# christopherkarani/Wax

Measured on NVIDIA H100. Metric: queries/sec cosine top-10 @ 10Mx384 fp32, higher is better.
Workload: dtype f32

## Files before the change

### wax_b200/csrc/waxvs_batch.cuh

```cuda
#pragma once
#include <cuda.h>
#include <cuda_bf16.h>

#include "waxvs_common.cuh"
#include "waxvs_scan.cuh"

namespace waxvs {

constexpr int kBatchM = 128;
constexpr int kBatchN = 128;
constexpr int kBatchKBlock = 32;
constexpr int kBatchKBlockBf16 = 64;
constexpr int kBatchRescore = 256;
constexpr int kBatchRescoreMax = 1024;
constexpr uint32_t kBatchABytes = kBatchM * 128u;
constexpr uint32_t kBatchBBytes = kBatchN * 128u;
constexpr uint32_t kBatchStageBytes = kBatchABytes + kBatchBBytes;
constexpr int kBatchStageSlots = 8;
constexpr uint32_t kBatchScoreStride = kBatchN + 8;
constexpr uint32_t kBatchScoreBytes = kBatchM * kBatchScoreStride * 4u;
constexpr int kBatchMaxStages = 6;
constexpr uint32_t kBatchSmemOptin = 227u * 1024u;
__host__ __device__ constexpr uint32_t batch_smem_bytes(int stages, int heap, uint32_t ares_kb = 0) {
    return ares_kb * kBatchABytes + stages * (ares_kb ? kBatchBBytes : kBatchStageBytes) + kBatchScoreBytes +
// ... 893 lines not shown
            }
        } else if (n_exact >= p.k) {
            const float dk = from_orderable_u32(static_cast<uint32_t>(ek[p.k - 1] >> 32));
            const float qn = s_sqrt_a2;
            const float scale = METRIC == kCosine ? qn : qn * __uint_as_float(*p.max_norm_bits);
            const float sk_exact = METRIC == kCosine ? (1.0f - dk) * qn : 1.0f - dk;
            const float acc_slack = static_cast<float>(p.dims) * 0x1p-23f * scale;
            const float ulp_slack = 0x1p-21f * fmaxf(1.0f, fabsf(dk)) * (METRIC == kCosine ? qn : 1.0f);
            const float eps = p.eps_rel * scale * 1.01f + acc_slack + ulp_slack + 1e-30f;
            if (excluded_any && (!(sk_exact > tau + eps) || !finite_f32(eps))) ok = 0;
            const float feps = kTf32Eps * scale * 1.01f + acc_slack + ulp_slack + 1e-30f;
            const float t = sk_exact - feps;
            tau_star = finite_f32(t) ? t - fabsf(t) * 0x1p-20f - 1e-30f : -INFINITY;
            const float feps16 = kBf16Eps * scale * 1.01f + acc_slack + ulp_slack + 1e-30f;
            const float t16 = sk_exact - feps16;
            tau_star16 = finite_f32(t16) ? t16 - fabsf(t16) * 0x1p-20f - 1e-30f : -INFINITY;
        } else if (excluded_any) {
            ok = 0;
        }
        if (METRIC != kL2 && (!(s_a2 >= 0x1p-126f) || !finite_f32(s_a2))) {
            ok = 0;
            tau_star = tau_star16 = -INFINITY;
        }
        p.ok[q] = ok;
        if (p.tau_star) { p.tau_star[q] = tau_star; p.tau_star[p.tau_stride + q] = tau_star16; }
    }
    ScanParams sp{};
    sp.out = p.out + static_cast<size_t>(q) * p.k;
    sp.frame_ids = p.frame_ids; sp.id_base = p.id_base; sp.row_offset = p.row_offset;
    for (uint32_t i = threadIdx.x; i < p.k; i += blockDim.x)
        write_candidate(sp, static_cast<int>(i), i < p.rescore ? ek[i] : WAXVS_KEY_NONE);
}

struct RescoreParams {
    const float *corpus, *query;
    uint32_t dims, k, n_nominees;
    const uint64_t *nominees;
    uint32_t *aux;
    const uint32_t *max_norm_bits;
    float rho_max;
    uint64_t *block_keys;
    uint32_t *ticket;
    uint32_t *work_counter;
    wax_vs_candidate *out;
    uint32_t *ok;
    const uint64_t *frame_ids;
    uint64_t id_base, row_offset;
    uint32_t tail_smem_bytes;
};

template <int METRIC>
__global__ void __launch_bounds__(512, 1) shadow_rescore_kernel(const RescoreParams p) {
    static_assert(METRIC == kCosine || METRIC == kDot, "the shadow route covers cosine and dot");
    extern __shared__ __align__(16) unsigned char rsm[];
    __shared__ float s_a2, s_sqrt_a2;
    const int warp = threadIdx.x >> 5, lane = threadIdx.x & 31, warps = blockDim.x >> 5;
    const int k = static_cast<int>(p.k);
    if (warp == 0) {
        float s0 = 0.f, s1 = 0.f, s2 = 0.f, s3 = 0.f;
        for (uint32_t base = 4u * lane; base < p.dims; base += 128u) {
            const float4 x = __ldg(reinterpret_cast<const float4 *>(p.query + base));
            s0 = __fmaf_rn(x.x, x.x, s0); s1 = __fmaf_rn(x.y, x.y, s1);
            s2 = __fmaf_rn(x.z, x.z, s2); s3 = __fmaf_rn(x.w, x.w, s3);
        }
        const float a2 = warp_butterfly_sum(__fadd_rn(__fadd_rn(s0, s1), __fadd_rn(s2, s3)));
        if (lane == 0) { s_a2 = a2; s_sqrt_a2 = __fsqrt_rn(a2); }
    }
    __shared__ ScanParams sp;
    for (uint32_t i = threadIdx.x; i < sizeof(ScanParams) / 4u; i += blockDim.x) reinterpret_cast<uint32_t *>(&sp)[i] = 0u;
    __syncthreads();
    if (threadIdx.x == 0) {
        sp.k = p.k; sp.block_keys = p.block_keys; sp.ticket = p.ticket; sp.out = p.out;
        sp.frame_ids = p.frame_ids; sp.id_base = p.id_base; sp.row_offset = p.row_offset;
        sp.tail_smem_bytes = p.tail_smem_bytes; sp.work_counter = p.work_counter;
    }
    __syncthreads();

    WarpTopK<1> tk;
    tk.init();
    const uint32_t stride = gridDim.x * warps * 4u;
    for (uint32_t i0 = (blockIdx.x * warps + warp) * 4u; i0 < p.n_nominees; i0 += stride) {
        uint64_t nk[4];
        const float *vp[4];
        float d[4];
#pragma unroll
        for (uint32_t r = 0; r < 4; ++r) {
            nk[r] = i0 + r < p.n_nominees ? p.nominees[i0 + r] : WAXVS_KEY_NONE;
            vp[r] = p.corpus + static_cast<size_t>(nk[r] == WAXVS_KEY_NONE ? 0u : static_cast<uint32_t>(nk[r])) * p.dims;
        }
        exact_row_distance_x4<METRIC>(p.query, vp, p.dims, s_a2, s_sqrt_a2, lane, d);
#pragma unroll
        for (uint32_t r = 0; r < 4; ++r) {
            if (nk[r] == WAXVS_KEY_NONE || !finite_f32(d[r])) continue;
            const uint64_t x = make_key(d[r], static_cast<uint32_t>(nk[r]));
            if (x < tk.thresh) tk.insert(x, lane, k);
        }
    }

    if (!finish_topk_select<1>(sp, tk, rsm)) return;
    __syncthreads();
    if (threadIdx.x != 0) return;
    const wax_vs_candidate kth = p.out[p.k - 1];
    const uint32_t cut = p.aux[0];
    const bool excluded_any = cut != WAXVS_UKEY_NONE;
    const float tau = excluded_any ? -from_orderable_u32(cut) : -INFINITY;
    const float rho_q = __uint_as_float(p.aux[1]);
    uint32_t ok = 1;
    if (kth.valid) {
        const float dk = kth.distance, qn = s_sqrt_a2;
        const float m = METRIC == kCosine ? 1.0f : __uint_as_float(*p.max_norm_bits);
        const float scale = qn * m;
        const float sk_exact = METRIC == kCosine ? (1.0f - dk) * qn : 1.0f - dk;
        const float coding = qn * p.rho_max + rho_q * ((METRIC == kCosine ? 1.0001f : m) + p.rho_max);
        const float acc_slack = static_cast<float>(p.dims) * 0x1p-23f * scale;
        const float ulp_slack = 0x1p-21f * fmaxf(1.0f, fabsf(dk)) * (METRIC == kCosine ? qn : 1.0f);
        const float eps = coding * 1.01f + acc_slack + ulp_slack + 1e-30f;
        if (excluded_any && (!(sk_exact > tau + eps) || !finite_f32(eps))) ok = 0;
    } else if (excluded_any) {
        ok = 0;
    }
    if (!(s_a2 >= 0x1p-126f) || !finite_f32(s_a2)) ok = 0;
    *p.ok = ok;
    p.aux[0] = WAXVS_UKEY_NONE;
    p.aux[2] = cut;
}

template <int METRIC>
__global__ void __launch_bounds__(256) filter_rescore_kernel(const float *corpus, const float *queries, uint32_t dims,
                                                             const uint32_t *cand_count, const uint32_t *cand_rows,
                                                             uint32_t cand_cap, uint64_t *keys) {
    const uint32_t q = blockIdx.y;
    const int lane = threadIdx.x & 31;
    const uint32_t n = min(cand_count[q], cand_cap);
    const uint32_t warps = (gridDim.x * blockDim.x) >> 5;
    uint32_t i = (blockIdx.x * blockDim.x + threadIdx.x) >> 5;
    if (i >= n) return;
    const float *qv = queries + static_cast<size_t>(q) * dims;
    float a2 = 0.0f, sqrt_a2 = 0.0f;
    if (METRIC == kCosine) {
        float s0 = 0.f, s1 = 0.f, s2 = 0.f, s3 = 0.f;
        for (uint32_t base = 4u * lane; base < dims; base += 128u) {
            const float x = __ldg(qv + base); s0 = __fmaf_rn(x, x, s0);
            if (base + 1 < dims) { const float y = __ldg(qv + base + 1); s1 = __fmaf_rn(y, y, s1); }
            if (base + 2 < dims) { const float z = __ldg(qv + base + 2); s2 = __fmaf_rn(z, z, s2); }
            if (base + 3 < dims) { const float w = __ldg(qv + base + 3); s3 = __fmaf_rn(w, w, s3); }
        }
        a2 = warp_butterfly_sum(__fadd_rn(__fadd_rn(s0, s1), __fadd_rn(s2, s3)));
        sqrt_a2 = __fsqrt_rn(a2);
    }
    for (uint32_t i0 = i; i0 < n; i0 += 4u * warps) {
        uint32_t rr[4];
        const float *vp[4];
        float d[4];
#pragma unroll
        for (uint32_t r = 0; r < 4; ++r) {
            const uint32_t j = i0 + r * warps;
            rr[r] = cand_rows[static_cast<size_t>(q) * cand_cap + (j < n ? j : i0)];
            vp[r] = corpus + static_cast<size_t>(rr[r]) * dims;
        }
// ... 41 lines not shown
```

### wax_b200/csrc/waxvs_engine.cu

```cuda
#include <cuda_runtime.h>

#include <algorithm>
#include <atomic>
#include <cstdarg>
#include <cstdio>
#include <cstring>
#include <mutex>
#include <new>
#include <shared_mutex>
#include <string>
#include <unordered_map>
#include <chrono>
#include <random>
#include <thread>
#include <unistd.h>
#include <cmath>
#include <vector>

#include "../../include/wax_vs_cuda.h"
#include "waxvs_common.cuh"
#include "waxvs_scan.cuh"
#include "waxvs_select.cuh"
#include "waxvs_synth.cuh"
#include "waxvs_batch.cuh"
// ... 523 lines not shown
static cudaError_t launch_shadow_scan(wax_vs_engine *e, const ScanParams &p, int grid, const TmaConfig &cfg, int metric,
                                      cudaStream_t s) {
#define WAXVS_CASE(Cv, Rv)                                                                                          \
    if (cfg.C == Cv && cfg.R == Rv)                                                                                 \
        return metric == kCosine ? launch_tma_inst<Cv, Rv, kCosine, 4, false, true>(e, p, grid, cfg, s)            \
                                 : launch_tma_inst<Cv, Rv, kDot, 4, false, true>(e, p, grid, cfg, s)
    WAXVS_CASE(1, 8); WAXVS_CASE(1, 16); WAXVS_CASE(2, 8); WAXVS_CASE(2, 16);
    WAXVS_CASE(3, 4); WAXVS_CASE(3, 8); WAXVS_CASE(3, 16); WAXVS_CASE(4, 4); WAXVS_CASE(4, 8);
    WAXVS_CASE(6, 2); WAXVS_CASE(6, 4); WAXVS_CASE(8, 2); WAXVS_CASE(8, 4); WAXVS_CASE(12, 2); WAXVS_CASE(12, 4);
#undef WAXVS_CASE
    return cudaErrorInvalidValue;
}
static cudaError_t launch_int8_scan(wax_vs_engine *e, const ScanParams &p, int grid, const TmaConfig &cfg, int metric,
                                   cudaStream_t s) {
#define WAXVS_CASE(Cv, Rv)                                                                                          \
    if (cfg.C == Cv && cfg.R == Rv)                                                                                 \
        return metric == kCosine ? launch_tma_inst<Cv, Rv, kCosine, 4, false, true, true>(e, p, grid, cfg, s)      \
                                 : launch_tma_inst<Cv, Rv, kDot, 4, false, true, true>(e, p, grid, cfg, s)
    WAXVS_CASE(1, 8); WAXVS_CASE(1, 16); WAXVS_CASE(2, 8); WAXVS_CASE(2, 16);
    WAXVS_CASE(3, 4); WAXVS_CASE(3, 8); WAXVS_CASE(3, 16); WAXVS_CASE(4, 4); WAXVS_CASE(4, 8);
    WAXVS_CASE(6, 4); WAXVS_CASE(6, 8); WAXVS_CASE(8, 4); WAXVS_CASE(12, 4);
#undef WAXVS_CASE
    return cudaErrorInvalidValue;
}
static bool pick_u4_config(const wax_vs_engine *e, TmaConfig *cfg) {
    if (!pick_tma_config(e, cfg, 1, 1)) return false;
    const int C = cfg->C, want_r = e->tune.u4_rows_per_step;
    const int r_hi = C <= 3 ? 16 : (C <= 6 ? 8 : 4), r_lo = C <= 3 ? 8 : 4;
    cfg->R = (want_r >= r_lo && want_r <= r_hi && (want_r & (want_r - 1)) == 0) ? want_r : r_hi;
    cfg->stages = e->tune.u4_stages > 0 ? e->tune.u4_stages : 3;
    cfg->warps = std::max(1, std::min(16, e->tune.u4_warps ? e->tune.u4_warps : 16));
    const size_t stage_bytes = static_cast<size_t>(cfg->R) * (e->dims / 2 + 4);
    cfg->smem = static_cast<size_t>(cfg->warps) * cfg->stages * (stage_bytes + 8 + 4) + static_cast<size_t>(cfg->warps) * 1024 + 16;
    return cfg->smem <= (e->smem_optin ? e->smem_optin : 232448) - 4096;
}
static cudaError_t launch_u4_scan(wax_vs_engine *e, const ScanParams &p, int grid, const TmaConfig &cfg, cudaStream_t s) {
#define WAXVS_CASE(Cv, Rv) \
    if (cfg.C == Cv && cfg.R == Rv) return launch_tma_inst<Cv, Rv, kDot, 4, false, true, false, true>(e, p, grid, cfg, s)
    WAXVS_CASE(1, 8); WAXVS_CASE(1, 16); WAXVS_CASE(2, 8); WAXVS_CASE(2, 16); WAXVS_CASE(3, 8); WAXVS_CASE(3, 16);
    WAXVS_CASE(4, 4); WAXVS_CASE(4, 8); WAXVS_CASE(6, 4); WAXVS_CASE(6, 8); WAXVS_CASE(8, 4); WAXVS_CASE(12, 4);
#undef WAXVS_CASE
    return cudaErrorInvalidValue;
}
static cudaError_t launch_ldg(const ScanParams &p, int grid, int metric, int mode, cudaStream_t s) {
    switch (metric * 3 + mode) {
        case 0: scan_ldg_kernel<kCosine, 1, false><<<grid, 256, 0, s>>>(p); break;
        case 1: scan_ldg_kernel<kCosine, 4, false><<<grid, 256, 0, s>>>(p); break;
        case 2: scan_ldg_kernel<kCosine, 1, true><<<grid, 256, 0, s>>>(p); break;
        case 3: scan_ldg_kernel<kDot, 1, false><<<grid, 256, 0, s>>>(p); break;
        case 4: scan_ldg_kernel<kDot, 4, false><<<grid, 256, 0, s>>>(p); break;
        case 5: scan_ldg_kernel<kDot, 1, true><<<grid, 256, 0, s>>>(p); break;
        case 6: scan_ldg_kernel<kL2, 1, false><<<grid, 256, 0, s>>>(p); break;
        case 7: scan_ldg_kernel<kL2, 4, false><<<grid, 256, 0, s>>>(p); break;
        default: scan_ldg_kernel<kL2, 1, true><<<grid, 256, 0, s>>>(p); break;
    }
    return cudaGetLastError();
}

static int32_t wait_host_flag(cudaStream_t stream, unsigned long long *flag_ptr, unsigned long long seq,
                              unsigned long long timeout_ns) {
    volatile unsigned long long *flag = flag_ptr;
    const auto t0 = std::chrono::steady_clock::now();
    uint32_t spins = 0;
    for (;;) {
        const unsigned long long v = *flag;
        if ((v & ~kShardErrorBit) == seq) {
            std::atomic_thread_fence(std::memory_order_acquire);
// ... 94 lines not shown
    *form = RouteForm::kBf16;
    TmaConfig cfg{};
    int32_t rc;
    if (!demoted && e->n_rows * e->dims * sizeof(float) >= e->tune.u4_scan_min_bytes && pick_u4_config(e, &cfg)) {
        if ((rc = ensure_coded_shadow(e, e->u4, stream))) return rc;
        if (e->u4.valid && std::isfinite(e->u4.eps_rel)) { *form = RouteForm::kU4; return WAX_VS_OK; }
    }
    bool int8 = false;
    if ((rc = int8_route_selected(e, stream, &int8))) return rc;
    if (int8) *form = RouteForm::kInt8;
    return WAX_VS_OK;
}

static int32_t enqueue_shadow_nominations(wax_vs_engine *e, SearchCtx *c, const ScanParams &p, const TmaConfig &cfg,
                                          cudaStream_t stream, uint64_t *launches, uint32_t *shape = nullptr,
                                          RouteForm form = RouteForm::kBf16) {
    const bool int8 = form == RouteForm::kInt8, u4 = form == RouteForm::kU4;
    int32_t rc;
    if (u4 && !c->d_u4_aux) {
        if ((rc = c->d_u4_aux.ensure(3, "4-bit route state"))) return rc;
        CUDA_TRY(cudaMemsetAsync(c->d_u4_aux, 0xFF, 3 * sizeof(uint32_t), stream));
    }
    const size_t u4_keys = static_cast<size_t>(std::max(e->tune.grid, e->sm_count)) * kU4CtaNominees;
    if ((rc = c->d_heaps.ensure(std::max(static_cast<size_t>(kShadowNominees) * kNomineeStride, u4 ? u4_keys : 0), "nominee keys")) ||
        (rc = c->d_ok.ensure(1, "proof flags")) || (!p.query && (rc = c->d_queries.ensure(e->dims, "query buffer"))))
        return rc;

    ScanParams sp = p;
    sp.corpus = u4 ? reinterpret_cast<const float *>(e->u4.codes.p)
                   : int8 ? reinterpret_cast<const float *>(e->i8.codes.p) : reinterpret_cast<const float *>(e->d_shadow.p);
    sp.row_scale = u4 ? e->u4.scale.p : int8 ? e->i8.scale.p : nullptr;
    sp.u4_aux = u4 ? c->d_u4_aux.p : nullptr;
    sp.k = kShadowNominees;
    sp.out = nullptr; sp.host_out = nullptr; sp.host_flag = nullptr;
    sp.nominees = c->d_heaps;
    sp.query_store = p.query ? nullptr : c->d_queries.p;
    sp.tail_select = e->tune.tail_select ? 1u : 0u;
    sp.tail_smem_bytes = static_cast<uint32_t>(static_cast<size_t>(cfg.warps) * cfg.stages * cfg.R * e->dims *
                                               (int8 ? 1 : sizeof(__nv_bfloat16)));
    const int grid = tma_grid(e, c, cfg, sp);
    if (u4) CUDA_TRY(launch_u4_scan(e, sp, grid, cfg, stream));
    else if (int8) CUDA_TRY(launch_int8_scan(e, sp, grid, cfg, e->similarity, stream));
    else CUDA_TRY(launch_shadow_scan(e, sp, grid, cfg, e->similarity, stream));

    if (u4) {
        RescoreParams rp{};
        rp.corpus = e->d_corpus; rp.query = p.query ? p.query : c->d_queries.p;
        rp.dims = e->dims; rp.k = p.k; rp.n_nominees = static_cast<uint32_t>(grid) * kU4CtaNominees;
        rp.nominees = c->d_heaps; rp.aux = c->d_u4_aux; rp.max_norm_bits = e->d_max_norm; rp.rho_max = e->u4.rho_max;
        rp.block_keys = c->d_block_keys; rp.ticket = c->d_ticket; rp.work_counter = sp.work_counter; rp.out = p.out; rp.ok = c->d_ok;
        rp.frame_ids = p.frame_ids; rp.id_base = p.id_base; rp.row_offset = p.row_offset;
        rp.tail_smem_bytes = static_cast<uint32_t>(grid) * p.k * sizeof(uint64_t);
        if (rp.tail_smem_bytes > 48u * 1024u) rp.tail_smem_bytes = 0;
        const auto kernel = e->similarity == WAX_VS_COSINE ? shadow_rescore_kernel<kCosine> : shadow_rescore_kernel<kDot>;
        kernel<<<grid, 512, rp.tail_smem_bytes, stream>>>(rp);
        CUDA_TRY(cudaGetLastError());
    } else {
    FinishParams fp{};
    fp.corpus = e->d_corpus; fp.queries = p.query ? p.query : c->d_queries.p;
    fp.n_rows = p.n_rows; fp.dims = e->dims; fp.n_queries = 1; fp.groups = 1; fp.slices = 1;
    fp.kprime = kShadowNominees; fp.k = p.k; fp.metric = e->similarity;
    fp.heaps = c->d_heaps; fp.max_norm_bits = e->d_max_norm;
    fp.out = p.out; fp.ok = c->d_ok;
    fp.frame_ids = p.frame_ids; fp.id_base = p.id_base; fp.row_offset = p.row_offset;
    fp.pow2_all = 512; fp.rescore = kShadowRescore; fp.eps_rel = int8 ? e->i8.eps_rel : kBf16Eps;
    const size_t fsmem = static_cast<size_t>(fp.pow2_all + fp.rescore) * sizeof(uint64_t);
    const auto kernel = e->similarity == WAX_VS_COSINE ? batch_finish_kernel<kCosine> : batch_finish_kernel<kDot>;
    CUDA_TRY(grant_smem(e, kernel, fsmem));
    kernel<<<1, 512, fsmem, stream>>>(fp);
    CUDA_TRY(cudaGetLastError());
    }
    *launches += 2;
    if (shape) {
        const uint32_t s[7] = {static_cast<uint32_t>(cfg.C), static_cast<uint32_t>(cfg.R), static_cast<uint32_t>(cfg.warps),
                               static_cast<uint32_t>(cfg.stages), static_cast<uint32_t>(grid), sp.chunk_steps, sp.tail_select};
        std::copy(s, s + 7, shape);
    }
    return WAX_VS_OK;
}

static int32_t enqueue_shadow_route(wax_vs_engine *e, SearchCtx *c, ScanParams &p, cudaStream_t stream, uint64_t *launches) {
    if (!shadow_route_applies(e)) return WAX_VS_OK;
    TmaConfig cfg{};
    if (!pick_tma_config(e, &cfg, 1, sizeof(__nv_bfloat16))) return WAX_VS_OK;
    int32_t rc;
    if (!c->h_proof_count) {
        if ((rc = c->d_proof_count.ensure(2, "proof counts")) || (rc = c->h_proof_count.ensure(2, "proof count mirror"))) return rc;
        CUDA_TRY(cudaMemsetAsync(c->d_proof_count, 0, 2 * sizeof(uint32_t), stream));
        c->h_proof_count[0] = c->h_proof_count[1] = 0;
        c->seen_failed = 0;
    }
    bool demoted;
    {
        std::lock_guard<std::mutex> pg(e->pool_mu);
        const uint32_t failed = *static_cast<volatile uint32_t *>(c->h_proof_count + 1);
        if (failed != c->seen_failed) {
            c->seen_failed = failed;
            if (c->last_u4) {
                if (e->u4_probing) e->u4_demote_window = std::min(e->u4_demote_window * 2, 1u << 20);
                e->u4_demoted = e->u4_demote_window;
            } else {
                e->shadow_scan_skip = kShadowSkipQueries;
            }
        } else if (c->last_u4 && e->u4_probing) {
            e->u4_demote_window = 16;
// ... 3582 lines not shown
```

### wax_b200/csrc/waxvs_scan.cuh

```cuda
#pragma once
#include "waxvs_common.cuh"
#include "waxvs_shard.cuh"
#include "../../include/wax_vs_cuda.h"

namespace waxvs {

constexpr int kInlineQueryFloats = 512;

struct ScanParams {
    const float *corpus;
    const float *query;
    uint32_t n_rows;
    uint32_t dims;
    uint32_t k;
    uint32_t stages;
    uint64_t *block_keys;
    uint32_t *ticket;
    wax_vs_candidate *out;
    uint32_t *dist_keys;
    const uint64_t *frame_ids;
    uint64_t id_base;
    uint64_t row_offset;
    uint32_t use_l2_hint;
    uint32_t chunk_steps;
    uint32_t *work_counter;
    const uint32_t *mask;
    wax_vs_candidate *host_out;
    unsigned long long *host_flag;
    unsigned long long host_seq;
    alignas(16) float query_inline[kInlineQueryFloats];
    uint32_t tail_select;
    uint32_t tail_smem_bytes;
    unsigned long long *trace;
    ShardParams shard;
    uint64_t *nominees;
    float *query_store;
    const uint32_t *proof_ok;
    uint32_t *proof_count;
    uint32_t *proof_count_host;
    const float *row_scale;
    uint32_t *u4_aux;
};

constexpr uint32_t kU4CtaNominees = 256;

constexpr int kNomineeStride = 128;

__device__ __forceinline__ bool row_allowed(const ScanParams &p, uint32_t row) {
    return p.mask == nullptr || ((__ldg(p.mask + (row >> 5)) >> (row & 31u)) & 1u) != 0u;
}

__device__ __forceinline__ void write_candidate(const ScanParams &p, int slot, uint64_t key) {
    wax_vs_candidate c;
    if (key == WAXVS_KEY_NONE) {
        c.distance = 0.0f; c.valid = 0; c.row = 0; c.frame_id = 0;
    } else {
        const uint32_t row = static_cast<uint32_t>(key);
        c.distance = from_orderable_u32(static_cast<uint32_t>(key >> 32));
        c.valid = 1;
        c.row = p.row_offset + row;
        c.frame_id = p.frame_ids ? p.frame_ids[row] : p.id_base + row;
    }
    p.out[slot] = c;
    if (p.host_out) p.host_out[slot] = c;
}

template <bool SHADOW>
__device__ __forceinline__ void write_slot(const ScanParams &p, int slot, uint64_t key) {
    if constexpr (SHADOW) p.nominees[static_cast<size_t>(slot == static_cast<int>(p.k) - 1 ? 0 : slot + 1) * kNomineeStride] = key;
    else write_candidate(p, slot, key);
}

__device__ __forceinline__ float4 bf16x4_to_float4(uint2 u) {
    return make_float4(__uint_as_float(u.x << 16), __uint_as_float(u.x & 0xFFFF0000u),
                       __uint_as_float(u.y << 16), __uint_as_float(u.y & 0xFFFF0000u));
}

__device__ __forceinline__ float4 int8x4_to_float4(uint32_t u) {
    constexpr float kBias = 8388736.0f;
    return make_float4(__fsub_rn(__uint_as_float(__byte_perm(u, 0x4B000000u, 0x7650)), kBias),
                       __fsub_rn(__uint_as_float(__byte_perm(u, 0x4B000000u, 0x7651)), kBias),
                       __fsub_rn(__uint_as_float(__byte_perm(u, 0x4B000000u, 0x7652)), kBias),
                       __fsub_rn(__uint_as_float(__byte_perm(u, 0x4B000000u, 0x7653)), kBias));
}

template <int H>
__device__ __forceinline__ void half_warp_reduce_scatter(int (&v)[H], int lane) {
    static_assert(H == 1 || H == 2 || H == 4 || H == 8, "H must be a power of two <= 8");
    int off = 8;
#pragma unroll
    for (int half = H / 2; half >= 1; half >>= 1, off >>= 1) {
        const bool upper = (lane & off) != 0;
#pragma unroll
        for (int j = 0; j < half; ++j) {
            const int send = upper ? v[j] : v[j + half];
            const int keep = upper ? v[j + half] : v[j];
            v[j] = keep + __shfl_xor_sync(WAXVS_FULL_MASK, send, off);
        }
    }
#pragma unroll
    for (; off >= 1; off >>= 1) v[0] += __shfl_xor_sync(WAXVS_FULL_MASK, v[0], off);
}

// ... 25 lines not shown
    }
    __syncthreads();
    if (!s_last) return;
    __threadfence();
    tk.init();
    constexpr int U = (E == 1) ? 4 : 2;
#pragma unroll 1
    for (uint32_t b0 = warp; b0 < gridDim.x; b0 += warps * U) {
        uint64_t other[U][E];
#pragma unroll
        for (int u = 0; u < U; ++u) {
            const uint32_t b = b0 + u * warps;
#pragma unroll
            for (int j = 0; j < E; ++j)
                other[u][j] = (b < gridDim.x) ? ld_cg_u64(p.block_keys + static_cast<size_t>(b) * W + j * 32 + lane)
                                              : WAXVS_KEY_NONE;
        }
#pragma unroll
        for (int u = 0; u < U; ++u) tk.merge_sorted(other[u], lane, k);
    }
    __syncthreads();
#pragma unroll
    for (int j = 0; j < E; ++j) lists[warp * W + j * 32 + lane] = tk.key[j];
    __syncthreads();
    if (warp == 0) {
#pragma unroll 1
        for (int w = 1; w < warps; ++w) {
            uint64_t other[E];
            load_list(lists + w * W, other);
            tk.merge_sorted(other, lane, k);
        }
#pragma unroll
        for (int j = 0; j < E; ++j)
            if (j * 32 + lane < k) write_slot<SHADOW>(p, j * 32 + lane, tk.key[j]);
        if (lane == 0) { *p.ticket = 0u; if (p.work_counter) *p.work_counter = 0u; }
        if (p.host_flag && !p.shard.world) {
            __threadfence_system();
            __syncwarp();
            if (lane == 0) st_release_sys_u64(p.host_flag, p.host_seq);
        }
    }
    if (p.shard.world) shard_exchange_cta(p.shard, p.out, p.k, reinterpret_cast<uint32_t *>(lists));
}

struct SelectScratch {
    uint32_t hist[256];
    uint64_t sel[128];
    uint32_t digit, k_rem, in_bin, n_sel;
    unsigned long long found;
};

template <typename ForEach>
__device__ __forceinline__ uint64_t block_select_kth(ForEach for_each, uint32_t k, SelectScratch *ss) {
    const uint32_t tid = threadIdx.x;
    uint64_t prefix = 0;
    uint32_t k_rem = k;
#pragma unroll 1
    for (int shift = 56; shift >= 0; shift -= 8) {
        for (uint32_t i = tid; i < 256u; i += blockDim.x) ss->hist[i] = 0;
        __syncthreads();
        const uint64_t want = (shift == 56) ? 0ull : (prefix >> (shift + 8));
        for_each([&](uint64_t key) {
            if (shift == 56 || (key >> (shift + 8)) == want) atomicAdd(&ss->hist[(key >> shift) & 255u], 1u);
        });
        __syncthreads();
        if (tid < 32) {
            uint32_t c[8], sum = 0;
// ... 1 lines not shown
            for (int i = 0; i < 8; ++i) { c[i] = ss->hist[tid * 8 + i]; sum += c[i]; }
            uint32_t incl = sum;
#pragma unroll
            for (int off = 1; off < 32; off <<= 1) {
                const uint32_t up = __shfl_up_sync(WAXVS_FULL_MASK, incl, off);
                if (static_cast<int>(tid) >= off) incl += up;
            }
            const uint32_t excl = incl - sum;
            if (excl < k_rem && k_rem <= incl) {
                uint32_t run = excl;
#pragma unroll
                for (int i = 0; i < 8; ++i) {
                    if (run < k_rem && k_rem <= run + c[i]) { ss->digit = tid * 8 + i; ss->k_rem = k_rem - run; ss->in_bin = c[i]; }
                    run += c[i];
                }
            }
        }
        __syncthreads();
        prefix |= static_cast<uint64_t>(ss->digit) << shift;
        k_rem = ss->k_rem;
        if (ss->in_bin == 1u && shift > 0) {
            const uint64_t top = prefix >> shift;
            for_each([&](uint64_t key) { if ((key >> shift) == top) ss->found = key; });
            __syncthreads();
            const uint64_t x = ss->found;
            __syncthreads();
            return x;
        }
    }
    return prefix;
}

template <int E, bool SHADOW = false>
__device__ __forceinline__ bool finish_topk_select(const ScanParams &p, WarpTopK<E> &tk, unsigned char *scratch) {
    __shared__ SelectScratch ss;
    __shared__ uint32_t s_last2;
    const uint32_t tid = threadIdx.x, nthr = blockDim.x, k = p.k;
    auto own_keys = [&](auto f) {
#pragma unroll
        for (int j = 0; j < E; ++j) f(tk.key[j]);
    };
    const uint64_t xa = block_select_kth(own_keys, k, &ss);
    if (tid == 0) ss.n_sel = 0;
    __syncthreads();
    uint64_t *mine = p.block_keys + static_cast<size_t>(blockIdx.x) * k;
#pragma unroll
    for (int j = 0; j < E; ++j)
        if (tk.key[j] != WAXVS_KEY_NONE && tk.key[j] <= xa) mine[atomicAdd(&ss.n_sel, 1u)] = tk.key[j];
    __syncthreads();
    for (uint32_t i = ss.n_sel + tid; i < k; i += nthr) mine[i] = WAXVS_KEY_NONE;
    __threadfence();
    __syncthreads();
    if (p.trace && tid == 0) atomicMax(p.trace + 2, global_timer_ns());
    if (tid == 0) s_last2 = (atomicAdd(p.ticket, 1u) == gridDim.x - 1) ? 1u : 0u;
    __syncthreads();
    if (!s_last2) return false;
    __threadfence();
    if (p.trace && tid == 0) p.trace[3] = global_timer_ns();
    const uint32_t total = gridDim.x * k;
    const bool staged = static_cast<size_t>(total) * sizeof(uint64_t) <= p.tail_smem_bytes;
    uint64_t *sk = reinterpret_cast<uint64_t *>(scratch);
    if (staged) {
        for (uint32_t i = tid; i < total; i += nthr) sk[i] = ld_cg_u64(p.block_keys + i);
        __syncthreads();
    }
    auto grid_keys = [&](auto f) {
        if (staged) { for (uint32_t i = tid; i < total; i += nthr) f(sk[i]); }
        else { for (uint32_t i = tid; i < total; i += nthr) f(ld_cg_u64(p.block_keys + i)); }
    };
    const uint64_t xb = block_select_kth(grid_keys, k, &ss);
    if (tid == 0) ss.n_sel = 0;
    __syncthreads();
    grid_keys([&](uint64_t key) { if (key != WAXVS_KEY_NONE && key <= xb) ss.sel[atomicAdd(&ss.n_sel, 1u)] = key; });
    __syncthreads();
    const uint32_t n_sel = ss.n_sel;
    for (uint32_t i = tid; i < k; i += nthr) {
        if (i < n_sel) {
            const uint64_t key = ss.sel[i];
            uint32_t rank = 0;
            for (uint32_t j = 0; j < n_sel; ++j) rank += ss.sel[j] < key ? 1u : 0u;
            write_slot<SHADOW>(p, static_cast<int>(rank), key);
        } else {
            write_slot<SHADOW>(p, static_cast<int>(i), WAXVS_KEY_NONE);
        }
    }
    if (p.host_flag && !p.shard.world) __threadfence_system();
    __syncthreads();
    if (tid == 0) {
        *p.ticket = 0u;
        if (p.work_counter) *p.work_counter = 0u;
        if (p.host_flag && !p.shard.world) st_release_sys_u64(p.host_flag, p.host_seq);
        if (p.trace) p.trace[4] = global_timer_ns();
    }
    if (p.shard.world) shard_exchange_cta(p.shard, p.out, p.k, reinterpret_cast<uint32_t *>(scratch));
    return true;
}

template <int E>
__device__ __forceinline__ void finish_u4_nominees(const ScanParams &p, WarpTopK<E> &tk) {
    __shared__ SelectScratch ss;
    __shared__ uint32_t s_cut;
    const uint32_t tid = threadIdx.x, nthr = blockDim.x;
    if (tid == 0) s_cut = WAXVS_UKEY_NONE;
    auto own_keys = [&](auto f) {
#pragma unroll
        for (int j = 0; j < E; ++j) f(tk.key[j]);
    };
    const uint64_t xa = block_select_kth(own_keys, kU4CtaNominees, &ss);
    if (tid == 0) ss.n_sel = 0;
    __syncthreads();
    uint64_t *mine = p.nominees + static_cast<size_t>(blockIdx.x) * kU4CtaNominees;
#pragma unroll
    for (int j = 0; j < E; ++j)
        if (tk.key[j] != WAXVS_KEY_NONE && tk.key[j] <= xa) mine[atomicAdd(&ss.n_sel, 1u)] = tk.key[j];
    if ((tid & 31u) == 0 && tk.thresh != WAXVS_KEY_NONE) atomicMin(&s_cut, static_cast<uint32_t>(tk.thresh >> 32));
    __syncthreads();
    for (uint32_t i = ss.n_sel + tid; i < kU4CtaNominees; i += nthr) mine[i] = WAXVS_KEY_NONE;
    if (tid == 0) {
        uint32_t cut = s_cut;
        if (xa != WAXVS_KEY_NONE) cut = min(cut, static_cast<uint32_t>(xa >> 32));
        if (cut != WAXVS_UKEY_NONE) atomicMin(p.u4_aux, cut);
    }
}

template <int C, int R, int METRIC, int E, bool EMIT, bool SHADOW = false, bool INT8 = false, bool U4 = false>
__global__ void __launch_bounds__(512, 1) scan_tma_kernel(const __grid_constant__ ScanParams p) {
    static_assert(!SHADOW || (C > 0 && METRIC != kL2 && !EMIT), "the shadow form covers the unrolled cosine / dot shapes");
    static_assert(!INT8 || (SHADOW && R >= 4), "the int8 form is a shadow form with 16-byte scale copies");
    static_assert(!U4 || (SHADOW && !INT8 && R >= 4 && E == 4), "the 4-bit form is a shadow form with 16-byte scale copies");
    constexpr bool SCALED = INT8 || U4;
    if constexpr (!SHADOW && !EMIT && E == 1 && METRIC != kL2) {
        if (p.proof_ok) {
            const bool proven = *p.proof_ok != 0u;
            if (blockIdx.x == 0) {
                if (threadIdx.x == 0) {
                    const uint32_t n = ++p.proof_count[proven ? 0 : 1];
                    *static_cast<volatile uint32_t *>(p.proof_count_host + (proven ? 0 : 1)) = n;
                }
                if (proven && p.host_flag) {
                    for (uint32_t i = threadIdx.x; i < p.k; i += blockDim.x) p.host_out[i] = p.out[i];
                    __threadfence_system();
                    __syncthreads();
                    if (threadIdx.x == 0) st_release_sys_u64(p.host_flag, p.host_seq);
                }
            }
            if (proven) return;
        }
    }
    const int D4 = C > 0 ? 32 * C : static_cast<int>(p.dims / 4u);
    const int CN = C > 0 ? C : (D4 + 31) / 32;
    const uint32_t ROW_BYTES = C > 0 ? (U4 ? 64u : INT8 ? 128u : SHADOW ? 256u : 512u) * C : p.dims * 4u;
    const uint32_t STAGE_BYTES = ROW_BYTES * R + (SCALED ? R * 4u : 0u);
    constexpr int LANES_PER_ROW = 32 / R;

    extern __shared__ __align__(128) unsigned char smem[];
    const int warp = threadIdx.x >> 5, lane = threadIdx.x & 31, warps = blockDim.x >> 5;
    const uint32_t stages = p.stages;
    unsigned char *ring = smem + static_cast<size_t>(warp) * stages * STAGE_BYTES;
    uint64_t *bars = reinterpret_cast<uint64_t *>(smem + static_cast<size_t>(warps) * stages * STAGE_BYTES) +
                     warp * stages;
    uint64_t *lists = reinterpret_cast<uint64_t *>(smem + static_cast<size_t>(warps) * stages * STAGE_BYTES) +
                      warps * stages;
    uint32_t *stage_step = reinterpret_cast<uint32_t *>(lists + warps * 32 * E) + warp * stages;
    float4 *qs = reinterpret_cast<float4 *>(reinterpret_cast<uint32_t *>(lists + warps * 32 * E) + warps * stages + 4);

    float4 q[C > 0 ? C : 1];
    const float4 *q4 = reinterpret_cast<const float4 *>(p.query);
    const float4 *qp = reinterpret_cast<const float4 *>(p.query_inline);
    auto load_q = [&](int i) -> float4 { return q4 ? __ldg(q4 + i) : qp[i]; };
    if (C > 0) {
#pragma unroll
        for (int c = 0; c < (C > 0 ? C : 1); ++c) q[c] = load_q(lane + 32 * c);
// ... 239 lines not shown
        else d = finish_l2(sum0[0]);
        if (SHADOW && !finite_f32(d)) d = -INFINITY;
        const bool leader = U4 ? (hl % (16 / H)) == 0 : (lane % LANES_PER_ROW) == 0;
        const bool ok = (my_row < p.n_rows) && (SHADOW || finite_f32(d));

        if (EMIT) {
            if (leader && my_row < p.n_rows)
                p.dist_keys[my_row] = (ok && row_allowed(p, my_row)) ? orderable_u32(d) : WAXVS_UKEY_NONE;
        } else {
            const uint64_t key = ok ? make_key(d, my_row) : WAXVS_KEY_NONE;
            const bool cand = leader && key < tk.thresh && row_allowed(p, my_row);
            uint32_t m = __ballot_sync(WAXVS_FULL_MASK, cand);
            if (E == 1) {
                while (m) {
                    const int src = __ffs(m) - 1;
                    m &= m - 1;
                    const uint64_t x = shfl_u64(key, src);
                    if (x < tk.thresh) tk.insert(x, lane, k);
                }
            } else if (m) {
                if (tk.npend + __popc(m) > 32) tk.flush(lane, k);
                while (m) {
                    const int src = __ffs(m) - 1;
                    m &= m - 1;
                    tk.park(shfl_u64(key, src), lane);
                }
            }
        }
    }

    if (p.trace && lane == 0) atomicMax(p.trace + 1, global_timer_ns());
    if (!EMIT) {
        if (E > 1) tk.flush(lane, k);
        if constexpr (U4) finish_u4_nominees<E>(p, tk);
        else if (p.tail_select) finish_topk_select<E, SHADOW>(p, tk, smem);
        else finish_topk<E, SHADOW>(p, tk, lists, warp, lane, warps);
    }
}

template <int METRIC, int E, bool EMIT>
__global__ void __launch_bounds__(256, 4) scan_ldg_kernel(const __grid_constant__ ScanParams p) {
    __shared__ uint64_t lists[8 * 32 * E];
    const int warp = threadIdx.x >> 5, lane = threadIdx.x & 31, warps = blockDim.x >> 5;
    const uint32_t dims = p.dims;
    const bool vec4 = (dims % 4u) == 0u;
    const uint32_t d4 = dims / 4u;

    float a2 = 0.0f, sqrt_a2 = 0.0f;
    if (METRIC == kCosine) {
        float s0 = 0.f, s1 = 0.f, s2 = 0.f, s3 = 0.f;
        for (uint32_t base = 4u * lane; base < dims; base += 128u) {
            const float x = __ldg(p.query + base);
            const float y = (base + 1 < dims) ? __ldg(p.query + base + 1) : 0.0f;
            const float z = (base + 2 < dims) ? __ldg(p.query + base + 2) : 0.0f;
            const float w = (base + 3 < dims) ? __ldg(p.query + base + 3) : 0.0f;
            s0 = __fmaf_rn(x, x, s0);
            if (base + 1 < dims) s1 = __fmaf_rn(y, y, s1);
            if (base + 2 < dims) s2 = __fmaf_rn(z, z, s2);
            if (base + 3 < dims) s3 = __fmaf_rn(w, w, s3);
        }
        a2 = warp_butterfly_sum(__fadd_rn(__fadd_rn(s0, s1), __fadd_rn(s2, s3)));
        sqrt_a2 = __fsqrt_rn(a2);
    }

    WarpTopK<E> tk;
    tk.init();
    const int k = static_cast<int>(p.k);
    const uint32_t total_warps = gridDim.x * warps;
// ... 57 lines not shown
```

Baseline: 1499.

## Fuse u4 shadow rescore into scan kernel tail with TMA row gather

```diff
diff --git a/wax_b200/csrc/waxvs_batch.cuh b/wax_b200/csrc/waxvs_batch.cuh
--- a/wax_b200/csrc/waxvs_batch.cuh
+++ b/wax_b200/csrc/waxvs_batch.cuh
@@ -949,99 +949,6 @@
         write_candidate(sp, static_cast<int>(i), i < p.rescore ? ek[i] : WAXVS_KEY_NONE);
 }
 
-struct RescoreParams {
-    const float *corpus, *query;
-    uint32_t dims, k, n_nominees;
-    const uint64_t *nominees;
-    uint32_t *aux;
-    const uint32_t *max_norm_bits;
-    float rho_max;
-    uint64_t *block_keys;
-    uint32_t *ticket;
-    uint32_t *work_counter;
-    wax_vs_candidate *out;
-    uint32_t *ok;
-    const uint64_t *frame_ids;
-    uint64_t id_base, row_offset;
-    uint32_t tail_smem_bytes;
-};
-
-template <int METRIC>
-__global__ void __launch_bounds__(512, 1) shadow_rescore_kernel(const RescoreParams p) {
-    static_assert(METRIC == kCosine || METRIC == kDot, "the shadow route covers cosine and dot");
-    extern __shared__ __align__(16) unsigned char rsm[];
-    __shared__ float s_a2, s_sqrt_a2;
-    const int warp = threadIdx.x >> 5, lane = threadIdx.x & 31, warps = blockDim.x >> 5;
-    const int k = static_cast<int>(p.k);
-    if (warp == 0) {
-        float s0 = 0.f, s1 = 0.f, s2 = 0.f, s3 = 0.f;
-        for (uint32_t base = 4u * lane; base < p.dims; base += 128u) {
-            const float4 x = __ldg(reinterpret_cast<const float4 *>(p.query + base));
-            s0 = __fmaf_rn(x.x, x.x, s0); s1 = __fmaf_rn(x.y, x.y, s1);
-            s2 = __fmaf_rn(x.z, x.z, s2); s3 = __fmaf_rn(x.w, x.w, s3);
-        }
-        const float a2 = warp_butterfly_sum(__fadd_rn(__fadd_rn(s0, s1), __fadd_rn(s2, s3)));
-        if (lane == 0) { s_a2 = a2; s_sqrt_a2 = __fsqrt_rn(a2); }
-    }
-    __shared__ ScanParams sp;
-    for (uint32_t i = threadIdx.x; i < sizeof(ScanParams) / 4u; i += blockDim.x) reinterpret_cast<uint32_t *>(&sp)[i] = 0u;
-    __syncthreads();
-    if (threadIdx.x == 0) {
-        sp.k = p.k; sp.block_keys = p.block_keys; sp.ticket = p.ticket; sp.out = p.out;
-        sp.frame_ids = p.frame_ids; sp.id_base = p.id_base; sp.row_offset = p.row_offset;
-        sp.tail_smem_bytes = p.tail_smem_bytes; sp.work_counter = p.work_counter;
-    }
-    __syncthreads();
-
-    WarpTopK<1> tk;
-    tk.init();
-    const uint32_t stride = gridDim.x * warps * 4u;
-    for (uint32_t i0 = (blockIdx.x * warps + warp) * 4u; i0 < p.n_nominees; i0 += stride) {
-        uint64_t nk[4];
-        const float *vp[4];
-        float d[4];
-#pragma unroll
-        for (uint32_t r = 0; r < 4; ++r) {
-            nk[r] = i0 + r < p.n_nominees ? p.nominees[i0 + r] : WAXVS_KEY_NONE;
-            vp[r] = p.corpus + static_cast<size_t>(nk[r] == WAXVS_KEY_NONE ? 0u : static_cast<uint32_t>(nk[r])) * p.dims;
-        }
-        exact_row_distance_x4<METRIC>(p.query, vp, p.dims, s_a2, s_sqrt_a2, lane, d);
-#pragma unroll
-        for (uint32_t r = 0; r < 4; ++r) {
-            if (nk[r] == WAXVS_KEY_NONE || !finite_f32(d[r])) continue;
-            const uint64_t x = make_key(d[r], static_cast<uint32_t>(nk[r]));
-            if (x < tk.thresh) tk.insert(x, lane, k);
-        }
-    }
-
-    if (!finish_topk_select<1>(sp, tk, rsm)) return;
-    __syncthreads();
-    if (threadIdx.x != 0) return;
-    const wax_vs_candidate kth = p.out[p.k - 1];
-    const uint32_t cut = p.aux[0];
-    const bool excluded_any = cut != WAXVS_UKEY_NONE;
-    const float tau = excluded_any ? -from_orderable_u32(cut) : -INFINITY;
-    const float rho_q = __uint_as_float(p.aux[1]);
-    uint32_t ok = 1;
-    if (kth.valid) {
-        const float dk = kth.distance, qn = s_sqrt_a2;
-        const float m = METRIC == kCosine ? 1.0f : __uint_as_float(*p.max_norm_bits);
-        const float scale = qn * m;
-        const float sk_exact = METRIC == kCosine ? (1.0f - dk) * qn : 1.0f - dk;
-        const float coding = qn * p.rho_max + rho_q * ((METRIC == kCosine ? 1.0001f : m) + p.rho_max);
-        const float acc_slack = static_cast<float>(p.dims) * 0x1p-23f * scale;
-        const float ulp_slack = 0x1p-21f * fmaxf(1.0f, fabsf(dk)) * (METRIC == kCosine ? qn : 1.0f);
-        const float eps = coding * 1.01f + acc_slack + ulp_slack + 1e-30f;
-        if (excluded_any && (!(sk_exact > tau + eps) || !finite_f32(eps))) ok = 0;
-    } else if (excluded_any) {
-        ok = 0;
-    }
-    if (!(s_a2 >= 0x1p-126f) || !finite_f32(s_a2)) ok = 0;
-    *p.ok = ok;
-    p.aux[0] = WAXVS_UKEY_NONE;
-    p.aux[2] = cut;
-}
-
 template <int METRIC>
 __global__ void __launch_bounds__(256) filter_rescore_kernel(const float *corpus, const float *queries, uint32_t dims,
                                                              const uint32_t *cand_count, const uint32_t *cand_rows,
diff --git a/wax_b200/csrc/waxvs_engine.cu b/wax_b200/csrc/waxvs_engine.cu
--- a/wax_b200/csrc/waxvs_engine.cu
+++ b/wax_b200/csrc/waxvs_engine.cu
@@ -579,7 +579,8 @@
     cfg->warps = std::max(1, std::min(16, e->tune.u4_warps ? e->tune.u4_warps : 16));
     const size_t stage_bytes = static_cast<size_t>(cfg->R) * (e->dims / 2 + 4);
     cfg->smem = static_cast<size_t>(cfg->warps) * cfg->stages * (stage_bytes + 8 + 4) + static_cast<size_t>(cfg->warps) * 1024 + 16;
-    return cfg->smem <= (e->smem_optin ? e->smem_optin : 232448) - 4096;
+    return cfg->warps * cfg->stages * stage_bytes >= e->dims * sizeof(float) &&
+           cfg->smem <= (e->smem_optin ? e->smem_optin : 232448) - 12288;
 }
 static cudaError_t launch_u4_scan(wax_vs_engine *e, const ScanParams &p, int grid, const TmaConfig &cfg, cudaStream_t s) {
 #define WAXVS_CASE(Cv, Rv) \
@@ -740,30 +741,24 @@
     sp.row_scale = u4 ? e->u4.scale.p : int8 ? e->i8.scale.p : nullptr;
     sp.u4_aux = u4 ? c->d_u4_aux.p : nullptr;
     sp.k = kShadowNominees;
-    sp.out = nullptr; sp.host_out = nullptr; sp.host_flag = nullptr;
     sp.nominees = c->d_heaps;
-    sp.query_store = p.query ? nullptr : c->d_queries.p;
     sp.tail_select = e->tune.tail_select ? 1u : 0u;
-    sp.tail_smem_bytes = static_cast<uint32_t>(static_cast<size_t>(cfg.warps) * cfg.stages * cfg.R * e->dims *
-                                               (int8 ? 1 : sizeof(__nv_bfloat16)));
+    if (u4) {
+        sp.u4_rows = e->d_corpus; sp.u4_k = p.k; sp.u4_cosine = e->similarity == WAX_VS_COSINE ? 1u : 0u;
+        sp.max_norm_bits = e->d_max_norm; sp.rho_max = e->u4.rho_max; sp.u4_ok = c->d_ok;
+        sp.tail_smem_bytes = static_cast<uint32_t>(cfg.warps * cfg.stages * cfg.R * (e->dims / 2 + 4));
+    } else {
+        sp.out = nullptr; sp.host_out = nullptr; sp.host_flag = nullptr;
+        sp.query_store = p.query ? nullptr : c->d_queries.p;
+        sp.tail_smem_bytes = static_cast<uint32_t>(static_cast<size_t>(cfg.warps) * cfg.stages * cfg.R * e->dims *
+                                                   (int8 ? 1 : sizeof(__nv_bfloat16)));
+    }
     const int grid = tma_grid(e, c, cfg, sp);
     if (u4) CUDA_TRY(launch_u4_scan(e, sp, grid, cfg, stream));
     else if (int8) CUDA_TRY(launch_int8_scan(e, sp, grid, cfg, e->similarity, stream));
     else CUDA_TRY(launch_shadow_scan(e, sp, grid, cfg, e->similarity, stream));
 
-    if (u4) {
-        RescoreParams rp{};
-        rp.corpus = e->d_corpus; rp.query = p.query ? p.query : c->d_queries.p;
-        rp.dims = e->dims; rp.k = p.k; rp.n_nominees = static_cast<uint32_t>(grid) * kU4CtaNominees;
-        rp.nominees = c->d_heaps; rp.aux = c->d_u4_aux; rp.max_norm_bits = e->d_max_norm; rp.rho_max = e->u4.rho_max;
-        rp.block_keys = c->d_block_keys; rp.ticket = c->d_ticket; rp.work_counter = sp.work_counter; rp.out = p.out; rp.ok = c->d_ok;
-        rp.frame_ids = p.frame_ids; rp.id_base = p.id_base; rp.row_offset = p.row_offset;
-        rp.tail_smem_bytes = static_cast<uint32_t>(grid) * p.k * sizeof(uint64_t);
-        if (rp.tail_smem_bytes > 48u * 1024u) rp.tail_smem_bytes = 0;
-        const auto kernel = e->similarity == WAX_VS_COSINE ? shadow_rescore_kernel<kCosine> : shadow_rescore_kernel<kDot>;
-        kernel<<<grid, 512, rp.tail_smem_bytes, stream>>>(rp);
-        CUDA_TRY(cudaGetLastError());
-    } else {
+    if (!u4) {
     FinishParams fp{};
     fp.corpus = e->d_corpus; fp.queries = p.query ? p.query : c->d_queries.p;
     fp.n_rows = p.n_rows; fp.dims = e->dims; fp.n_queries = 1; fp.groups = 1; fp.slices = 1;
@@ -778,7 +773,7 @@
     kernel<<<1, 512, fsmem, stream>>>(fp);
     CUDA_TRY(cudaGetLastError());
     }
-    *launches += 2;
+    *launches += u4 ? 1 : 2;
     if (shape) {
         const uint32_t s[7] = {static_cast<uint32_t>(cfg.C), static_cast<uint32_t>(cfg.R), static_cast<uint32_t>(cfg.warps),
                                static_cast<uint32_t>(cfg.stages), static_cast<uint32_t>(grid), sp.chunk_steps, sp.tail_select};
diff --git a/wax_b200/csrc/waxvs_scan.cuh b/wax_b200/csrc/waxvs_scan.cuh
--- a/wax_b200/csrc/waxvs_scan.cuh
+++ b/wax_b200/csrc/waxvs_scan.cuh
@@ -40,6 +40,12 @@
     uint32_t *proof_count_host;
     const float *row_scale;
     uint32_t *u4_aux;
+    const float *u4_rows;
+    uint32_t u4_k;
+    uint32_t u4_cosine;
+    const uint32_t *max_norm_bits;
+    float rho_max;
+    uint32_t *u4_ok;
 };
 
 constexpr uint32_t kU4CtaNominees = 256;
@@ -50,7 +56,7 @@
     return p.mask == nullptr || ((__ldg(p.mask + (row >> 5)) >> (row & 31u)) & 1u) != 0u;
 }
 
-__device__ __forceinline__ void write_candidate(const ScanParams &p, int slot, uint64_t key) {
+__device__ __forceinline__ void write_candidate(const ScanParams &p, int slot, uint64_t key, bool to_host = true) {
     wax_vs_candidate c;
     if (key == WAXVS_KEY_NONE) {
         c.distance = 0.0f; c.valid = 0; c.row = 0; c.frame_id = 0;
@@ -62,13 +68,13 @@
         c.frame_id = p.frame_ids ? p.frame_ids[row] : p.id_base + row;
     }
     p.out[slot] = c;
-    if (p.host_out) p.host_out[slot] = c;
+    if (to_host && p.host_out) p.host_out[slot] = c;
 }
 
 template <bool SHADOW>
-__device__ __forceinline__ void write_slot(const ScanParams &p, int slot, uint64_t key) {
+__device__ __forceinline__ void write_slot(const ScanParams &p, int slot, uint64_t key, bool to_host) {
     if constexpr (SHADOW) p.nominees[static_cast<size_t>(slot == static_cast<int>(p.k) - 1 ? 0 : slot + 1) * kNomineeStride] = key;
-    else write_candidate(p, slot, key);
+    else write_candidate(p, slot, key, to_host);
 }
 
 __device__ __forceinline__ float4 bf16x4_to_float4(uint2 u) {
@@ -160,7 +166,7 @@
         }
 #pragma unroll
         for (int j = 0; j < E; ++j)
-            if (j * 32 + lane < k) write_slot<SHADOW>(p, j * 32 + lane, tk.key[j]);
+            if (j * 32 + lane < k) write_slot<SHADOW>(p, j * 32 + lane, tk.key[j], true);
         if (lane == 0) { *p.ticket = 0u; if (p.work_counter) *p.work_counter = 0u; }
         if (p.host_flag && !p.shard.world) {
             __threadfence_system();
@@ -228,10 +234,12 @@
 }
 
 template <int E, bool SHADOW = false>
-__device__ __forceinline__ bool finish_topk_select(const ScanParams &p, WarpTopK<E> &tk, unsigned char *scratch) {
+__device__ __forceinline__ bool finish_topk_select(const ScanParams &p, WarpTopK<E> &tk, unsigned char *scratch, uint32_t k,
+                                                   bool to_host = true) {
     __shared__ SelectScratch ss;
     __shared__ uint32_t s_last2;
-    const uint32_t tid = threadIdx.x, nthr = blockDim.x, k = p.k;
+    const uint32_t tid = threadIdx.x, nthr = blockDim.x;
+    const bool deliver = to_host && p.host_flag && !p.shard.world;
     auto own_keys = [&](auto f) {
 #pragma unroll
         for (int j = 0; j < E; ++j) f(tk.key[j]);
@@ -275,17 +283,17 @@
             const uint64_t key = ss.sel[i];
             uint32_t rank = 0;
             for (uint32_t j = 0; j < n_sel; ++j) rank += ss.sel[j] < key ? 1u : 0u;
-            write_slot<SHADOW>(p, static_cast<int>(rank), key);
+            write_slot<SHADOW>(p, static_cast<int>(rank), key, to_host);
         } else {
-            write_slot<SHADOW>(p, static_cast<int>(i), WAXVS_KEY_NONE);
-        }
-    }
-    if (p.host_flag && !p.shard.world) __threadfence_system();
+            write_slot<SHADOW>(p, static_cast<int>(i), WAXVS_KEY_NONE, to_host);
+        }
+    }
+    if (deliver) __threadfence_system();
     __syncthreads();
     if (tid == 0) {
         *p.ticket = 0u;
         if (p.work_counter) *p.work_counter = 0u;
-        if (p.host_flag && !p.shard.world) st_release_sys_u64(p.host_flag, p.host_seq);
+        if (deliver) st_release_sys_u64(p.host_flag, p.host_seq);
         if (p.trace) p.trace[4] = global_timer_ns();
     }
     if (p.shard.world) shard_exchange_cta(p.shard, p.out, p.k, reinterpret_cast<uint32_t *>(scratch));
@@ -293,7 +301,7 @@
 }
 
 template <int E>
-__device__ __forceinline__ void finish_u4_nominees(const ScanParams &p, WarpTopK<E> &tk) {
+__device__ __forceinline__ uint32_t finish_u4_nominees(const ScanParams &p, WarpTopK<E> &tk, uint64_t *keys) {
     __shared__ SelectScratch ss;
     __shared__ uint32_t s_cut;
     const uint32_t tid = threadIdx.x, nthr = blockDim.x;
@@ -308,14 +316,143 @@
     uint64_t *mine = p.nominees + static_cast<size_t>(blockIdx.x) * kU4CtaNominees;
 #pragma unroll
     for (int j = 0; j < E; ++j)
-        if (tk.key[j] != WAXVS_KEY_NONE && tk.key[j] <= xa) mine[atomicAdd(&ss.n_sel, 1u)] = tk.key[j];
+        if (tk.key[j] != WAXVS_KEY_NONE && tk.key[j] <= xa) {
+            const uint32_t at = atomicAdd(&ss.n_sel, 1u);
+            mine[at] = tk.key[j];
+            keys[at] = tk.key[j];
+        }
     if ((tid & 31u) == 0 && tk.thresh != WAXVS_KEY_NONE) atomicMin(&s_cut, static_cast<uint32_t>(tk.thresh >> 32));
     __syncthreads();
-    for (uint32_t i = ss.n_sel + tid; i < kU4CtaNominees; i += nthr) mine[i] = WAXVS_KEY_NONE;
+    const uint32_t n = ss.n_sel;
+    for (uint32_t i = n + tid; i < kU4CtaNominees; i += nthr) mine[i] = WAXVS_KEY_NONE;
     if (tid == 0) {
         uint32_t cut = s_cut;
         if (xa != WAXVS_KEY_NONE) cut = min(cut, static_cast<uint32_t>(xa >> 32));
         if (cut != WAXVS_UKEY_NONE) atomicMin(p.u4_aux, cut);
+    }
+    __syncthreads();
+    return n;
+}
+
+template <int C>
+__device__ __forceinline__ void finish_u4_rescore(const ScanParams &p, const uint64_t *keys, uint32_t n, unsigned char *ring,
+                                                  uint32_t ring_bytes) {
+    __shared__ __align__(8) uint64_t s_bar;
+    __shared__ uint32_t s_rows[kU4CtaNominees], s_fill, s_ok;
+    constexpr uint32_t ROW_BYTES = 512u * C;
+    const int warp = threadIdx.x >> 5, lane = threadIdx.x & 31, warps = blockDim.x >> 5;
+    const bool cosine = p.u4_cosine != 0u;
+    const int k = static_cast<int>(p.u4_k);
+    const float4 *q4 = reinterpret_cast<const float4 *>(p.query);
+    const float4 *qp = reinterpret_cast<const float4 *>(p.query_inline);
+    float4 q[C];
+    float s0 = 0.f, s1 = 0.f, s2 = 0.f, s3 = 0.f;
+#pragma unroll
+    for (int c = 0; c < C; ++c) {
+        q[c] = q4 ? __ldg(q4 + lane + 32 * c) : qp[lane + 32 * c];
+        s0 = __fmaf_rn(q[c].x, q[c].x, s0); s1 = __fmaf_rn(q[c].y, q[c].y, s1);
+        s2 = __fmaf_rn(q[c].z, q[c].z, s2); s3 = __fmaf_rn(q[c].w, q[c].w, s3);
+    }
+    const float a2 = warp_butterfly_sum(__fadd_rn(__fadd_rn(s0, s1), __fadd_rn(s2, s3)));
+    const float sqrt_a2 = __fsqrt_rn(a2);
+    if (threadIdx.x == 0) {
+        mbar_init(&s_bar, 1);
+        mbar_fence_init();
+    }
+    __syncthreads();
+
+    WarpTopK<1> ek;
+    ek.init();
+    const uint32_t per_fill = min(ring_bytes / ROW_BYTES, kU4CtaNominees);
+    uint32_t parity = 0, pos = 0;
+#pragma unroll 1
+    for (;; parity ^= 1u) {
+        if (warp == 0) {
+            const uint32_t cut = *static_cast<volatile uint32_t *>(p.u4_aux);
+            uint32_t rows = 0;
+            while (pos < n && rows < per_fill) {
+                const uint32_t i = pos + lane;
+                const bool keep = i < n && static_cast<uint32_t>(keys[i] >> 32) < cut;
+                const uint32_t m = __ballot_sync(WAXVS_FULL_MASK, keep);
+                const uint32_t slot = rows + __popc(m & ((1u << lane) - 1u));
+                if (keep && slot < per_fill) s_rows[slot] = static_cast<uint32_t>(keys[i]);
+                const uint32_t over = __ballot_sync(WAXVS_FULL_MASK, keep && slot >= per_fill);
+                pos = over ? pos + __ffs(over) - 1 : pos + 32u;
+                rows = min(rows + __popc(m), per_fill);
+            }
+            if (lane == 0) {
+                s_fill = rows;
+                if (rows) mbar_arrive_expect_tx(&s_bar, rows * ROW_BYTES);
+            }
+            __syncwarp();
+            for (uint32_t j = lane; j < rows; j += 32u)
+                bulk_copy_g2s(ring + j * ROW_BYTES, p.u4_rows + static_cast<size_t>(s_rows[j]) * (128 * C), ROW_BYTES, &s_bar);
+        }
+        __syncthreads();
+        const uint32_t rows = s_fill;
+        if (rows == 0) break;
+        mbar_wait_parity(&s_bar, parity);
+#pragma unroll 1
+        for (uint32_t j = warp; j < rows; j += warps) {
+            const float4 *v = reinterpret_cast<const float4 *>(ring + j * ROW_BYTES);
+            float a0 = 0.f, a1 = 0.f, a2_ = 0.f, a3 = 0.f, b0 = 0.f, b1 = 0.f, b2 = 0.f, b3 = 0.f;
+#pragma unroll
+            for (int c = 0; c < C; ++c) {
+                const float4 x = v[lane + 32 * c];
+                a0 = __fmaf_rn(q[c].x, x.x, a0); a1 = __fmaf_rn(q[c].y, x.y, a1);
+                a2_ = __fmaf_rn(q[c].z, x.z, a2_); a3 = __fmaf_rn(q[c].w, x.w, a3);
+                if (cosine) {
+                    b0 = __fmaf_rn(x.x, x.x, b0); b1 = __fmaf_rn(x.y, x.y, b1);
+                    b2 = __fmaf_rn(x.z, x.z, b2); b3 = __fmaf_rn(x.w, x.w, b3);
+                }
+            }
+            const float ab = warp_butterfly_sum(__fadd_rn(__fadd_rn(a0, a1), __fadd_rn(a2_, a3)));
+            const float d = cosine ? finish_cos(ab, a2, sqrt_a2, warp_butterfly_sum(__fadd_rn(__fadd_rn(b0, b1), __fadd_rn(b2, b3))))
+                                   : finish_dot(ab);
+            if (!finite_f32(d)) continue;
+            const uint64_t x = make_key(d, s_rows[j]);
+            if (x < ek.thresh) ek.insert(x, lane, k);
+        }
+        __syncthreads();
+    }
+
+    if (!finish_topk_select<1>(p, ek, ring, p.u4_k, false)) return;
+    __syncthreads();
+    if (threadIdx.x == 0) {
+        const wax_vs_candidate kth = p.out[p.u4_k - 1];
+        const uint32_t cut = *static_cast<volatile uint32_t *>(p.u4_aux);
+        const bool excluded_any = cut != WAXVS_UKEY_NONE;
+        const float tau = excluded_any ? -from_orderable_u32(cut) : -INFINITY;
+        const float rho_q = __uint_as_float(static_cast<volatile uint32_t *>(p.u4_aux)[1]);
+        uint32_t ok = 1;
+        if (kth.valid) {
+            const float dk = kth.distance, qn = sqrt_a2;
+            const float m = cosine ? 1.0f : __uint_as_float(*p.max_norm_bits);
+            const float scale = qn * m;
+            const float sk_exact = cosine ? (1.0f - dk) * qn : 1.0f - dk;
+            const float coding = qn * p.rho_max + rho_q * ((cosine ? 1.0001f : m) + p.rho_max);
+            const float acc_slack = static_cast<float>(p.dims) * 0x1p-23f * scale;
+            const float ulp_slack = 0x1p-21f * fmaxf(1.0f, fabsf(dk)) * (cosine ? qn : 1.0f);
+            const float eps = coding * 1.01f + acc_slack + ulp_slack + 1e-30f;
+            if (excluded_any && (!(sk_exact > tau + eps) || !finite_f32(eps))) ok = 0;
+        } else if (excluded_any) {
+            ok = 0;
+        }
+        if (!(a2 >= 0x1p-126f) || !finite_f32(a2)) ok = 0;
+        s_ok = ok;
+        p.u4_aux[0] = WAXVS_UKEY_NONE;
+        p.u4_aux[2] = cut;
+    }
+    __syncthreads();
+    const bool deliver = s_ok && p.host_flag;
+    if (deliver) {
+        for (uint32_t i = threadIdx.x; i < p.u4_k; i += blockDim.x) p.host_out[i] = p.out[i];
+        __threadfence_system();
+    }
+    __syncthreads();
+    if (threadIdx.x == 0) {
+        *p.u4_ok = deliver ? 2u : s_ok;
+        if (deliver) st_release_sys_u64(p.host_flag, p.host_seq);
     }
 }
 
@@ -327,13 +464,14 @@
     constexpr bool SCALED = INT8 || U4;
     if constexpr (!SHADOW && !EMIT && E == 1 && METRIC != kL2) {
         if (p.proof_ok) {
-            const bool proven = *p.proof_ok != 0u;
+            const uint32_t flag = *p.proof_ok;
+            const bool proven = flag != 0u;
             if (blockIdx.x == 0) {
                 if (threadIdx.x == 0) {
                     const uint32_t n = ++p.proof_count[proven ? 0 : 1];
                     *static_cast<volatile uint32_t *>(p.proof_count_host + (proven ? 0 : 1)) = n;
                 }
-                if (proven && p.host_flag) {
+                if (proven && flag != 2u && p.host_flag) {
                     for (uint32_t i = threadIdx.x; i < p.k; i += blockDim.x) p.host_out[i] = p.out[i];
                     __threadfence_system();
                     __syncthreads();
@@ -639,8 +777,11 @@
     if (p.trace && lane == 0) atomicMax(p.trace + 1, global_timer_ns());
     if (!EMIT) {
         if (E > 1) tk.flush(lane, k);
-        if constexpr (U4) finish_u4_nominees<E>(p, tk);
-        else if (p.tail_select) finish_topk_select<E, SHADOW>(p, tk, smem);
+        if constexpr (U4) {
+            __shared__ uint64_t nominees[kU4CtaNominees];
+            const uint32_t n = finish_u4_nominees<E>(p, tk, nominees);
+            finish_u4_rescore<C>(p, nominees, n, smem, static_cast<uint32_t>(warps) * stages * STAGE_BYTES);
+        } else if (p.tail_select) finish_topk_select<E, SHADOW>(p, tk, smem, p.k);
         else finish_topk<E, SHADOW>(p, tk, lists, warp, lane, warps);
     }
 }
```

After: 1519, median of 6. 1.4% higher.
